# int-brain-lab/mtscomp

Hardware: AMD Instinct MI355X
Metric: compress + decompress GB/s (raw int16) (higher is better)
Workload: dtype int16

## Files before the change

mtscomp_amd/csrc/deflate.hip:

```cpp
#include <stdlib.h>

#include <mutex>

#include "deflate_dev.h"
#include "op_rank.h"

namespace mts {

#ifndef MTS_SORT_WAVES
#define MTS_SORT_WAVES 8
#endif
#ifndef MTS_SORT_KPL
#define MTS_SORT_KPL 12
#endif
constexpr int SORT_WAVES = MTS_SORT_WAVES;
constexpr int SORT_KPL = MTS_SORT_KPL;
constexpr int SORT_NT = SORT_WAVES * 64;
#ifndef MTS_SORT_B1
#define MTS_SORT_B1 7
#endif
constexpr int SORT_B1 = MTS_SORT_B1;
constexpr int SORT_B2 = 15 - SORT_B1;
#ifndef MTS_SORT_SCRAMBLE
#define MTS_SORT_SCRAMBLE 0
#endif
__device__ __forceinline__ u32 sort_hash(u32 b012)
{
    u32 h = hash_of(b012);
#if MTS_SORT_SCRAMBLE
    h ^= h >> 8;
    h = (h * 0x5bd1u) & 0x7fffu;
    h ^= h >> 7;
#endif
    return h;
}
#ifndef MTS_SORT_SWZ
#define MTS_SORT_SWZ 1
#endif
__device__ __forceinline__ u32 cslot(u32 d) { return MTS_SORT_SWZ ? d ^ (d >> 5) : d; }

template <int NB>
__device__ __forceinline__ void bin_offsets(u32 (*cnt)[256], u32 *tot)
{
    constexpr int NBIN = 1 << NB;
    const int wave = threadIdx.x >> 6, lane = threadIdx.x & 63;
    const u32 cs = cslot(threadIdx.x);
    if (threadIdx.x < NBIN) {
        u32 run = 0;
        for (int w = 0; w < SORT_WAVES; w++) { const u32 c = cnt[w][cs]; cnt[w][cs] = run; run += c; }
        tot[threadIdx.x] = run;
    }
    __syncthreads();
    if (wave == 0) {
        u32 v[4], sum = 0;
#pragma unroll
        for (int k = 0; k < 4; k++) { v[k] = (lane * 4 + k < NBIN) ? tot[lane * 4 + k] : 0; sum += v[k]; }
        u32 total;
// ... 112 lines not shown

struct OpTile;
__device__ __forceinline__ bool op_two_pass(const OpTile *ot, u32 tile);
__global__ __launch_bounds__(SORT_NT) void k_hash_sort(const u8 *__restrict__ stream, const TileDesc *__restrict__ tiles,
                                                    u32 *__restrict__ tmp, u32 *__restrict__ sorted, int lane_ordered,
                                                    const OpTile *__restrict__ only )
{
    if (only && !op_two_pass(only, blockIdx.x)) return;
    const TileDesc td = tiles[blockIdx.x];
    __shared__ u32 cnt[SORT_WAVES][256];
    __shared__ u32 cnt2[SORT_WAVES][1 << SORT_B2];
    __shared__ u32 tot[256];
    __shared__ u32 stg[SORT_WAVES * 2 * 64 * SORT_KPL];
    __shared__ u32 dlt[SORT_WAVES * 256];
    if (td.wlen == 0) return;
    const u8 *s = stream + td.stream_off + td.w;
    const u32 wlen = td.wlen;
    const int wave = threadIdx.x >> 6, lane = threadIdx.x & 63;
    const u32 per = (((wlen + SORT_WAVES - 1) / SORT_WAVES) + 63) & ~63u;
    const u32 per_magic = per > 64 ? 0xffffffffu / (per >> 6) + 1 : 0;
    for (int i = threadIdx.x; i < SORT_WAVES * 256; i += SORT_NT) (&cnt[0][0])[i] = 0;
    for (int i = threadIdx.x; i < SORT_WAVES * (1 << SORT_B2); i += SORT_NT) (&cnt2[0][0])[i] = 0;
    __syncthreads();
    {
        const u32 beg = min((u32)wave * per, wlen), end = min(beg + per, wlen);
        constexpr int CK = 8;
        if (beg < end) {
            u32 vn[CK];
#pragma unroll
            for (int k = 0; k < CK; k++) vn[k] = gld_u32_unaligned(s, min(beg + lane + 64 * k, end - 1));
            for (u32 i0 = beg + lane; i0 < end; i0 += 64 * CK) {
                u32 v[CK];
#pragma unroll
                for (int k = 0; k < CK; k++) { v[k] = vn[k]; vn[k] = gld_u32_unaligned(s, min(i0 + 64 * CK + 64 * k, end - 1)); }
#pragma unroll
                for (int k = 0; k < CK; k++) if (i0 + 64 * k < end) atomicAdd(&cnt[wave][cslot(sort_hash(v[k]) & ((1u << SORT_B1) - 1))], 1u);
            }
        }
    }
    __syncthreads();
    u32 *tmp_t = tmp + td.sorted_off, *out_t = sorted + td.sorted_off;
    auto next_counts = [&]() {
        for (int i = threadIdx.x; i < SORT_WAVES * (1 << SORT_B2); i += SORT_NT) { cnt[i >> SORT_B2][i & ((1 << SORT_B2) - 1)] = cnt2[i >> SORT_B2][i & ((1 << SORT_B2) - 1)]; cnt2[i >> SORT_B2][i & ((1 << SORT_B2) - 1)] = 0; }
        __syncthreads();
    };
    bin_offsets<SORT_B1>(cnt, tot);
    rank_pass<SORT_B1, true, 0, SORT_B2>(s, nullptr, tmp_t, wlen, per, cnt, cnt2, per_magic, lane_ordered, stg, dlt);
    next_counts();
    bin_offsets<SORT_B2>(cnt, tot);
    rank_pass<SORT_B2, false, 0, 0>(s, tmp_t, out_t, wlen, per, cnt, cnt2, per_magic, lane_ordered, stg, dlt);
}


#ifndef MTS_OP_SLICE
#define MTS_OP_SLICE 8192
#endif
constexpr int OP_SLICE = MTS_OP_SLICE;
constexpr int OP_TILE_SLICES = WIN / OP_SLICE;
#ifndef MTS_OP_WAVES
#define MTS_OP_WAVES 16
#endif
constexpr int OP_WAVES = MTS_OP_WAVES;
constexpr int OP_NT = OP_WAVES * 64;
constexpr int OP_KPL = OP_SLICE / (OP_WAVES * 64);
constexpr int OP_LMAX = 1024;
constexpr int OP_MIN_KEYS = 2 * OP_SLICE;
constexpr int OP_ROW_WORDS = 512 + 1024;
#ifndef MTS_OP_LIVE_PARTS
#define MTS_OP_LIVE_PARTS 8
#endif
constexpr int OP_LIVE_PARTS = MTS_OP_LIVE_PARTS;
struct OpTile {
    uint2 bp[1024];
    u32 live, two_pass;
    u32 pad[62];
};
__device__ __forceinline__ bool op_two_pass(const OpTile *ot, u32 tile) { return ot[tile].two_pass != 0; }
__device__ __forceinline__ u32 op_slices(u32 wlen) { return (wlen + OP_SLICE - 1) / OP_SLICE; }
__device__ __forceinline__ bool op_tile_part(int n_tiles, u32 parts, u32 &tile, u32 &part)
{
    const u32 xcd = blockIdx.x & 7, jb = blockIdx.x >> 3;
    tile = (jb / parts) * 8 + xcd; part = jb % parts;
    return tile < (u32)n_tiles;
}
static unsigned op_grid(int n_tiles, unsigned parts) { return 8u * (((unsigned)n_tiles + 7) / 8) * parts; }

typedef u32 u32x2_a4 __attribute__((ext_vector_type(2), aligned(4)));
__device__ __forceinline__ u32x2_a4 op_load8(const u8 *s, u32 p) { return *(const __attribute__((address_space(1))) u32x2_a4 *)(u64)(s + p); }
__device__ __forceinline__ u32 op_hash_at(u32x2_a4 x, int k ) { return sort_hash(k ? __builtin_amdgcn_alignbyte(x.y, x.x, (u32)k) : x.x); }

__global__ __launch_bounds__(512) void k_op_live(const u8 *__restrict__ stream, const TileDesc *__restrict__ tiles, int n_tiles, OpTile *__restrict__ ot)
{
    __shared__ u32 bm[1024];
    u32 tile, part;
    if (!op_tile_part(n_tiles, OP_LIVE_PARTS, tile, part)) return;
    const TileDesc td = tiles[tile];
    if (td.wlen < (u32)OP_MIN_KEYS) return;
    const u32 per = ((td.wlen + OP_LIVE_PARTS - 1) / OP_LIVE_PARTS + 3) & ~3u, beg = min(part * per, td.wlen), end = min(beg + per, td.wlen);
    if (beg >= end) return;
    const u8 *s = stream + td.stream_off + td.w;
    for (int i = threadIdx.x; i < 1024; i += 512) bm[i] = 0;
    __syncthreads();
    constexpr int U = 8;
    for (u32 i0 = beg + 4 * threadIdx.x; i0 < end; i0 += 4 * 512 * U) {
        u32x2_a4 v[U];
#pragma unroll
        for (int k = 0; k < U; k++) v[k] = op_load8(s, min(i0 + 4u * 512 * k, (end - 1) & ~3u));
#pragma unroll
        for (int k = 0; k < U; k++)
#pragma unroll
            for (int q = 0; q < 4; q++)
                if (i0 + 4u * 512 * k + q < end) {
                    const u32 h = op_hash_at(v[k], q), bit = 1u << (h & 31);
                    if (!(bm[h >> 5] & bit)) atomicOr(&bm[h >> 5], bit);
                }
    }
    __syncthreads();
    for (int i = threadIdx.x; i < 1024; i += 512) if (bm[i]) atomicOr(&ot[tile].bp[i].x, bm[i]);
}

__global__ __launch_bounds__(1024) void k_op_prefix(const TileDesc *__restrict__ tiles, OpTile *__restrict__ ot)
{
    __shared__ u32 wsum[16];
    const u32 tile = blockIdx.x, w = threadIdx.x;
    const u32 c = (u32)__builtin_popcount(ot[tile].bp[w].x);
    u32 tot;
    const u32 ex = wave_excl_scan_u32(c, tot);
    if ((w & 63) == 0) wsum[w >> 6] = tot;
    __syncthreads();
    u32 before = 0, all = 0;
    for (u32 q = 0; q < 16; q++) { if (q < (w >> 6)) before += wsum[q]; all += wsum[q]; }
    ot[tile].bp[w].y = before + ex;
    if (w == 0) { ot[tile].live = all; ot[tile].two_pass = (tiles[tile].wlen < (u32)OP_MIN_KEYS || all > (u32)OP_LMAX) ? 1u : 0u; }
}

__device__ __forceinline__ u32 op_bucket(const uint2 *bp, u32 h)
{
    const uint2 e = bp[h >> 5];
    return e.y + (u32)__builtin_popcount(e.x & ((1u << (h & 31)) - 1u));
}

constexpr int OP_CNT_NT = 512;
__global__ __launch_bounds__(OP_CNT_NT) void k_op_count(const u8 *__restrict__ stream, const TileDesc *__restrict__ tiles, int n_tiles,
                                                        const OpTile *__restrict__ ot, u32 *__restrict__ scratch)
{
    __shared__ uint2 bp[1024];
    __shared__ u32 cnt[OP_LMAX];
    u32 tile, slice;
    if (!op_tile_part(n_tiles, OP_TILE_SLICES, tile, slice)) return;
    if (ot[tile].two_pass) return;
    const TileDesc td = tiles[tile];
    if (slice >= op_slices(td.wlen)) return;
    const u8 *s = stream + td.stream_off + td.w;
    for (int i = threadIdx.x; i < 1024; i += OP_CNT_NT) { bp[i] = ot[tile].bp[i]; cnt[i] = 0; }
    const u32 beg = slice * OP_SLICE, end = min(beg + (u32)OP_SLICE, td.wlen);
    constexpr int U = OP_SLICE / (4 * OP_CNT_NT);
    static_assert(OP_SLICE % (4 * OP_CNT_NT) == 0, "whole loads");
    u32x2_a4 v[U];
#pragma unroll
    for (int k = 0; k < U; k++) v[k] = op_load8(s, min(beg + 4u * (OP_CNT_NT * k + threadIdx.x), (end - 1) & ~3u));
    __syncthreads();
#pragma unroll
    for (int k = 0; k < U; k++)
#pragma unroll
        for (int q = 0; q < 4; q++)
            if (beg + 4u * (OP_CNT_NT * k + threadIdx.x) + q < end) atomicAdd(&cnt[op_bucket(bp, op_hash_at(v[k], q))], 1u);
    __syncthreads();
    u16 *row = (u16 *)(scratch + td.sorted_off + (size_t)slice * OP_ROW_WORDS);
    for (int i = threadIdx.x; i < 512; i += OP_CNT_NT) ((u32 *)row)[i] = cnt[2 * i] | (cnt[2 * i + 1] << 16);
}

__global__ __launch_bounds__(1024) void k_op_scan(const TileDesc *__restrict__ tiles, const OpTile *__restrict__ ot, u32 *__restrict__ scratch)
{
    __shared__ u32 wsum[16];
    const u32 tile = blockIdx.x, b = threadIdx.x;
    if (ot[tile].two_pass) return;
    const TileDesc td = tiles[tile];
    const u32 ns = op_slices(td.wlen);
    u32 *rows = scratch + td.sorted_off;
    u32 c[OP_TILE_SLICES], total = 0;
#pragma unroll
    for (int sl = 0; sl < OP_TILE_SLICES; sl++) c[sl] = (u32)sl < ns ? ((const u16 *)(rows + (size_t)sl * OP_ROW_WORDS))[b] : 0u;
#pragma unroll
    for (int sl = 0; sl < OP_TILE_SLICES; sl++) total += c[sl];
    u32 tot;
    const u32 ex = wave_excl_scan_u32(total, tot);
    if ((b & 63) == 0) wsum[b >> 6] = tot;
    __syncthreads();
    u32 run = ex;
    for (u32 q = 0; q < (b >> 6); q++) run += wsum[q];
#pragma unroll
    for (int sl = 0; sl < OP_TILE_SLICES; sl++) {
        if ((u32)sl < ns) rows[(size_t)sl * OP_ROW_WORDS + 512 + b] = run;
        run += c[sl];
    }
}

__global__ __launch_bounds__(OP_NT) void k_op_scatter(const u8 *__restrict__ stream, const TileDesc *__restrict__ tiles, int n_tiles,
                                                    const OpTile *__restrict__ ot, const u32 *__restrict__ scratch, u32 *__restrict__ sorted)
{
    __shared__ uint2 bp[1024];
    __shared__ u32 D[OP_LMAX];
    __shared__ u32 cw[OP_WAVES][OP_LMAX / 2];
    __shared__ u32 S[OP_SLICE];
    __shared__ u32 wsum[OP_WAVES];
    static_assert(OP_LMAX <= (1 << (32 - REL_BITS)) && OP_SLICE < 65536 && OP_SLICE % (OP_WAVES * 64) == 0, "position and bucket share a word; places in a slice are 16-bit");
    u32 tile, slice;
    if (!op_tile_part(n_tiles, OP_TILE_SLICES, tile, slice)) return;
    if (ot[tile].two_pass) return;
    const TileDesc td = tiles[tile];
    if (slice >= op_slices(td.wlen)) return;
    const u8 *s = stream + td.stream_off + td.w;
    const int wave = threadIdx.x >> 6, lane = threadIdx.x & 63;
    const u32 *row = scratch + td.sorted_off + (size_t)slice * OP_ROW_WORDS;
    for (int i = threadIdx.x; i < 1024; i += OP_NT) { bp[i] = ot[tile].bp[i]; D[i] = row[512 + i]; }
    for (int i = threadIdx.x; i < OP_WAVES * (OP_LMAX / 2); i += OP_NT) (&cw[0][0])[i] = 0;
    const u32 s0 = slice * OP_SLICE, beg = s0 + (u32)wave * (OP_SLICE / OP_WAVES), end = min(s0 + (u32)OP_SLICE, td.wlen);
    u32 v[OP_KPL];
#pragma unroll
    for (int k = 0; k < OP_KPL; k++) v[k] = gld_u32_unaligned(s, min(beg + 64u * k + lane, td.wlen - 1));
    __syncthreads();
    static_assert(OP_LMAX <= (1 << OP_ID_BITS) && OP_KPL * 64 <= (1 << (32 - OP_ID_BITS)), "bucket and rank share a word");
    u32 idr[OP_KPL];
#pragma unroll
    for (int k = 0; k < OP_KPL; k++) {
        const u32 id = op_bucket(bp, sort_hash(v[k]));
        idr[k] = id;
        if (beg + 64u * k + lane < end) idr[k] = op_pack_rank(id, atomicAdd(&cw[wave][op_cw_word(id)], op_cw_one(id)));
    }
    __syncthreads();
    {
        const int j = threadIdx.x & (OP_LMAX / 2 - 1);
        const bool mine = threadIdx.x < OP_LMAX / 2;
        u32 c[OP_WAVES], tot = 0;
#pragma unroll
        for (int w = 0; w < OP_WAVES; w++) { c[w] = mine ? cw[w][j] : 0u; tot += c[w]; }
        const u32 c0 = tot & 0xffffu, c1 = tot >> 16;
        u32 wtot;
        const u32 ex = wave_excl_scan_u32(c0 + c1, wtot);
        if (lane == 0) wsum[wave] = wtot;
        __syncthreads();
        u32 st0 = ex;
        for (int w = 0; w < wave; w++) st0 += wsum[w];
        const u32 st1 = st0 + c0;
        u32 run = st0 | (st1 << 16);
        if (mine) {
#pragma unroll
// ... 12 lines not shown
        }
    }
    __syncthreads();
    u32 *out = sorted + td.sorted_off;
    const u32 nk = end - s0;
#pragma unroll
    for (int k = 0; k < OP_KPL; k++) {
        const u32 j = threadIdx.x + (u32)OP_NT * k;
        if (j < nk) { const u32 e = S[j]; out[D[e >> REL_BITS] + j] = e; }
    }
}

static int lds_lane_ordered()
{
    static std::mutex mu;
    static int cached[64];
    static bool init = false;
    std::lock_guard<std::mutex> lk(mu);
    if (!init) { for (int i = 0; i < 64; i++) cached[i] = -1; init = true; }
    int dev = 0;
    if (hipGetDevice(&dev) != hipSuccess || dev < 0 || dev >= 64) return 0;
    if (cached[dev] >= 0) return cached[dev];
    u32 *d_bad = nullptr, h_bad = 1;
    if (hipMalloc(&d_bad, 4) != hipSuccess) return 0;
    if (hipMemset(d_bad, 0, 4) == hipSuccess) {
        hipLaunchKernelGGL(k_probe_lds_order, dim3(64), dim3(1024), 0, 0, d_bad, 512);
        if (hipMemcpy(&h_bad, d_bad, 4, hipMemcpyDeviceToHost) != hipSuccess) h_bad = 1;
    }
    (void)hipFree(d_bad);
    cached[dev] = h_bad == 0 ? 1 : 0;
    return cached[dev];
}

__global__ void k_inject_disorder(const u8 *__restrict__ stream, const TileDesc *__restrict__ tiles, u32 *__restrict__ sorted)
{
    const TileDesc td = tiles[0];
    const u8 *s = stream + td.stream_off + td.w;
    u32 *sk = sorted + td.sorted_off;
    for (u32 i = 0; i + 1 < td.wlen; i++) {
        const u32 a = sk[i], b = sk[i + 1];
        if (hash_of(gld_u32_unaligned(s, a & REL_MASK)) == hash_of(gld_u32_unaligned(s, b & REL_MASK)) && (b & REL_MASK) >= td.a - td.w) { sk[i] = b; sk[i + 1] = a; return; }
    }
}

size_t hash_sort_ws_bytes(int n_tiles) { return (size_t)(n_tiles + 1) * sizeof(OpTile); }

int launch_hash_sort(hipStream_t st, const u8 *d_stream, const TileDesc *d_tiles, int n_tiles, u32 *d_tmp, u32 *d_sorted, int force_ballot, void *d_ws)
{
    if (n_tiles == 0) return MTS_OK;
    const int ordered = (force_ballot == 1 || getenv("MTS_SORT_BALLOT")) ? 0 : lds_lane_ordered();
    static const bool two_pass_only = getenv("MTS_SORT_TWO_PASS") != nullptr;
    if (ordered && d_ws && !two_pass_only) {
        OpTile *ot = (OpTile *)d_ws;
        MTS_HIP(hipMemsetAsync(ot, 0, sizeof(OpTile) * (size_t)n_tiles, st));
        hipLaunchKernelGGL(k_op_live, dim3(op_grid(n_tiles, OP_LIVE_PARTS)), dim3(512), 0, st, d_stream, d_tiles, n_tiles, ot);
        hipLaunchKernelGGL(k_op_prefix, dim3(n_tiles), dim3(1024), 0, st, d_tiles, ot);
        hipLaunchKernelGGL(k_hash_sort, dim3(n_tiles), dim3(SORT_NT), 0, st, d_stream, d_tiles, d_tmp, d_sorted, ordered, (const OpTile *)ot);
        hipLaunchKernelGGL(k_op_count, dim3(op_grid(n_tiles, OP_TILE_SLICES)), dim3(OP_CNT_NT), 0, st, d_stream, d_tiles, n_tiles, (const OpTile *)ot, d_tmp);
        hipLaunchKernelGGL(k_op_scan, dim3(n_tiles), dim3(1024), 0, st, d_tiles, (const OpTile *)ot, d_tmp);
        hipLaunchKernelGGL(k_op_scatter, dim3(op_grid(n_tiles, OP_TILE_SLICES)), dim3(OP_NT), 0, st, d_stream, d_tiles, n_tiles, (const OpTile *)ot, (const u32 *)d_tmp, d_sorted);
    } else
        hipLaunchKernelGGL(k_hash_sort, dim3(n_tiles), dim3(SORT_NT), 0, st, d_stream, d_tiles, d_tmp, d_sorted, ordered, (const OpTile *)nullptr);
    if (force_ballot == 2) hipLaunchKernelGGL(k_inject_disorder, dim3(1), dim3(1), 0, st, d_stream, d_tiles, d_sorted);
    MTS_HIP(hipGetLastError());
    return MTS_OK;
}


typedef u32 u32x4_v __attribute__((ext_vector_type(4)));
typedef u32 u32x4_a4 __attribute__((ext_vector_type(4), aligned(4)));
typedef const __attribute__((address_space(1))) u32 *gptr_u32c;
typedef const __attribute__((address_space(1))) u32x4_v *gptr_uint4;
typedef const __attribute__((address_space(1))) u32x4_a4 *gptr_uint4_a4;
template <bool AHEAD, class RDU, class RD, class RDQ>
__device__ __forceinline__ u32 lazy_step(RDU &&rdu , RD &&rd, RDQ &&rdq, u32 p0, u32 n, const LevelCfg &cfg, u32 &mpos, u32 &mlen, u32 &mdist,
                                         u32 &mside )
{
    u32 p = p0;
    mside = 0;
    const u32 e0 = rdu(p);
    u32 e1 = 0, e2 = 0, e3 = 0;
    if (AHEAD) { e1 = rdu(p + 1); e2 = rdu(p + 2); e3 = rdu(p + 3); }
    u32 len = te_len(e0), dist = te_dist(e0);
    if (len == MIN_MATCH && dist > (u32)TOO_FAR) len = 0;
    if (len < MIN_MATCH) { mpos = p0; mlen = 0; mdist = 0; return p0 + 1; }
    for (;;) {
        const u32 q = p + 1;
        if (q < n && len < (u32)cfg.lazy) {
            u32 d;
            if (AHEAD) { d = q == p0 + 1 ? e1 : q == p0 + 2 ? e2 : e3; if (q > p0 + 3) d = rd(q); }
            else d = rd(q);
            u32 side = 0;
            if (len >= (u32)cfg.good) {
                if (d & TE_QNONE) d = 0;
                else if (d & TE_QSIDE) { d = rdq(q); side = 1; }
            }
            const u32 dl = te_len(d);
            if (dl > len) { p = q; len = dl; dist = te_dist(d); mside = side; continue; }
        }
        break;
    }
    mpos = p; mlen = len; mdist = dist;
    return p + len;
}
#define MTS_PARSE_GLOBAL_READERS(T, TQ)                                 \
    auto rd = [&](u32 q) -> u32 { return (T)[q]; };                     \
    auto rdq = [&](u32 q) -> u32 { return (TQ)[q]; };

constexpr int PARSE_WIN = 32;
constexpr int PARSE_AHEAD = 4;
constexpr int PARSE_ROW = PARSE_WIN + PARSE_AHEAD;
constexpr int PARSE_WIN_PITCH = PARSE_ROW + 1;
// ... 1636 lines not shown
```

mtscomp_amd/csrc/transform.hip:

```cpp
#include <stdlib.h>

#include "common.h"

namespace mts {


__device__ __forceinline__ u64 wave_sum_u64(u64 v)
{
#pragma unroll
    for (int off = 32; off > 0; off >>= 1) {
        u32 lo = __shfl_down((u32)v, off, 64), hi = __shfl_down((u32)(v >> 32), off, 64);
        v += ((u64)hi << 32) | lo;
    }
    return v;
}

__device__ __forceinline__ void block_sum2(u64 &a, u64 &b, u64 *sh )
{
    a = wave_sum_u64(a);
    b = wave_sum_u64(b);
    const int wave = threadIdx.x >> 6, lane = threadIdx.x & 63, nw = blockDim.x >> 6;
    if (lane == 0) { sh[wave] = a; sh[4 + wave] = b; }
    __syncthreads();
    if (threadIdx.x == 0) {
// ... 647 lines not shown
                const u32 v = (tt < tt_rows && t0 + tt < nt) ? (u32)d[(u64)c * nt + t0 + tt] : 0u;
                const u32 x = wave_incl_scan_dpp32(v) + run;
                if (tt < tt_rows) tile[tt * pitch + c] = (T)x;
                run = (u32)__builtin_amdgcn_readlane((int)x, 63);
            }
        }
    }
    __syncthreads();
    const int nrow = (int)min((long)tt_rows, nt - t0);
    T *out = (T *)(outb + out_off[chunk]) + t0 * nc;
    const long e_n = (long)nrow * nc;
    if ((((u64)out) & 15) == 0 && sizeof(T) <= 4) {
        constexpr int VW = 16 / (int)sizeof(T);
        const long n_full = e_n / VW;
        uint4 *oq = (uint4 *)out;
        for (long i = threadIdx.x; i < n_full; i += 256) {
            u32 r = __umulhi((u32)i * VW, nc_magic), c = (u32)i * VW - r * nc;
            u32 w[4] = {0, 0, 0, 0};
#pragma unroll
            for (int j = 0; j < VW; j++) {
                w[j / EPD] |= (u32)tile[r * pitch + c] << (8 * sizeof(T) * (j % EPD));
                if (++c == (u32)nc) { c = 0; r++; }
            }
            oq[i] = make_uint4(w[0], w[1], w[2], w[3]);
        }
        for (long e = n_full * VW + threadIdx.x; e < e_n; e += 256) {
            const u32 r = __umulhi((u32)e, nc_magic), c = (u32)e - r * nc;
            out[e] = tile[r * pitch + c];
        }
    } else if ((((u64)out) & 3) == 0) {
        u32 *od = (u32 *)out;
        for (long i = threadIdx.x; i * EPD < e_n; i += 256) {
            u32 v = 0;
            bool full = true;
#pragma unroll
            for (int j = 0; j < EPD; j++) {
                const u32 e = (u32)i * EPD + j;
                if (e < e_n) {
                    const u32 r = __umulhi(e, nc_magic), c = e - r * nc;
                    v |= (u32)tile[r * pitch + c] << (8 * sizeof(T) * j);
                } else full = false;
            }
            if (full) od[i] = v;
            else for (int j = 0; j < EPD; j++) if ((long)i * EPD + j < e_n) out[i * EPD + j] = (T)(v >> (8 * sizeof(T) * j));
        }
    } else {
        for (long i = threadIdx.x; i < e_n; i += 256) {
            const u32 r = __umulhi((u32)i, nc_magic), c = (u32)i - r * nc;
            out[i] = tile[r * pitch + c];
        }
    }
}

template <typename T>
static int run_cumsum_rows(hipStream_t st, const u8 *stream, u8 *out, const u64 *d_stream_off, const u64 *d_out_off,
                            const u32 *d_rows, const int *d_status, int n_chunks, u32 max_rows, int nc, u32 *sums)
{
    const int tt = rows_tile(nc, (int)sizeof(T)), pitch = rows_pitch(nc, (int)sizeof(T));
    const size_t lds = (size_t)tt * pitch * sizeof(T);
    const int rc = ensure_dynamic_lds((const void *)k_cumsum_rows<T>, ROWS_LDS_LIMIT);
    if (rc) return rc;
    const int ntile = (max_rows + tt - 1) / tt;
    dim3 grid(xcd_row_grid(ntile, n_chunks));
    hipLaunchKernelGGL(k_rows_sums<T>, grid, dim3(256), 0, st, stream, d_stream_off, d_rows, d_status, nc, tt, ntile, sums);
    hipLaunchKernelGGL(k_rows_scan, dim3((nc + 63) / 64, n_chunks), dim3(64 * ROWS_SCAN_PARTS), 0, st, d_rows, d_status, nc, tt, ntile, sums);
    hipLaunchKernelGGL(k_cumsum_rows<T>, grid, dim3(256), lds, st, stream, out, d_stream_off, d_out_off, d_rows, d_status, nc, tt, pitch,
                       0xffffffffu / (u32)nc + 1, ntile, sums);
    return MTS_OK;
}

static int segr_for(int itemsize) { return itemsize <= 2 ? 256 : itemsize == 4 ? 128 : 64; }

size_t cumsum_scratch_bytes(int n_chunks, u32 max_rows, int n_channels)
{
    const size_t seg = (size_t)n_chunks * ((max_rows + 63) / 64 + 1) * n_channels * sizeof(u64);
    const size_t til = (size_t)n_chunks * ((max_rows + 15) / 16 + 1) * n_channels * sizeof(u32);
    return (seg > til ? seg : til) + 256;
}

int launch_cumsum_transpose(hipStream_t st, const void *d_stream, void *d_out, const u64 *d_stream_off,
                            const u64 *d_out_off, const u32 *d_rows, const int *d_status, int n_chunks,
                            u32 max_rows, int n_channels, int itemsize, int flags, void *d_segsums)
{
    if (n_chunks == 0 || max_rows == 0) return MTS_OK;
    const u8 *s = (const u8 *)d_stream;
    u8 *o = (u8 *)d_out;
    u64 *ss = (u64 *)d_segsums;
    (void)segr_for;
    if (flags & MTS_FLAG_FLOAT) {
        if (itemsize == 4) return run_cumsum_float<float>(st, s, o, d_stream_off, d_out_off, d_rows, d_status, n_chunks, max_rows, n_channels, flags);
        if (itemsize == 8) return run_cumsum_float<double>(st, s, o, d_stream_off, d_out_off, d_rows, d_status, n_chunks, max_rows, n_channels, flags);
        return MTS_E_ARG;
    }
    if (flags == (MTS_FLAG_TIME_DIFF | MTS_FLAG_ORDER_F) && itemsize <= 4 && n_channels >= 2 && rows_tile(n_channels, itemsize) && !getenv("MTS_K12_GENERIC")) {
        int rc;
        switch (itemsize) {
        case 1: rc = run_cumsum_rows<u8>(st, s, o, d_stream_off, d_out_off, d_rows, d_status, n_chunks, max_rows, n_channels, (u32 *)ss); break;
        case 2: rc = run_cumsum_rows<u16>(st, s, o, d_stream_off, d_out_off, d_rows, d_status, n_chunks, max_rows, n_channels, (u32 *)ss); break;
        default: rc = run_cumsum_rows<u32>(st, s, o, d_stream_off, d_out_off, d_rows, d_status, n_chunks, max_rows, n_channels, (u32 *)ss); break;
        }
        if (rc) return rc;
        MTS_HIP(hipGetLastError());
        return MTS_OK;
    }
    switch (itemsize) {
    case 1: return run_cumsum<u8, 256>(st, s, o, d_stream_off, d_out_off, d_rows, d_status, n_chunks, max_rows, n_channels, flags, ss);
    case 2: return run_cumsum<u16, 256>(st, s, o, d_stream_off, d_out_off, d_rows, d_status, n_chunks, max_rows, n_channels, flags, ss);
    case 4: return run_cumsum<u32, 128>(st, s, o, d_stream_off, d_out_off, d_rows, d_status, n_chunks, max_rows, n_channels, flags, ss);
    case 8: return run_cumsum<u64, 64>(st, s, o, d_stream_off, d_out_off, d_rows, d_status, n_chunks, max_rows, n_channels, flags, ss);
    default: return MTS_E_ARG;
// ... 92 lines not shown
```

Before: 36.11.

## Fuse live-bitmap, prefix, count and scan into one per-tile planner kernel

Replaces four kernels plus a memset (k_op_live, k_op_prefix, k_op_count, k_op_scan) with a single k_op_plan that builds the live-hash bitmap, prefixes it, counts per-slice bucket occupancy in LDS with 16-bit packed counters, and writes the slice offsets for the scatter. It also computes hash word/bit directly from the key without the full sort_hash when scrambling is off, and software-pipelines the loads. This removes launch overhead and global round-trips for bitmap and count rows. In exchange each tile is handled by only one 1024-thread block, so there is less parallelism than the old slice-parallel count, and a large dynamic LDS footprint limits occupancy.

```diff
diff --git a/mtscomp_amd/csrc/deflate.hip b/mtscomp_amd/csrc/deflate.hip
--- a/mtscomp_amd/csrc/deflate.hip
+++ b/mtscomp_amd/csrc/deflate.hip
@@ -3,6 +3,7 @@
 #include <mutex>
 
 #include "deflate_dev.h"
+#include "op_plan.h"
 #include "op_rank.h"
 
 namespace mts {
@@ -221,31 +222,19 @@
 }
 
 
-#ifndef MTS_OP_SLICE
-#define MTS_OP_SLICE 8192
-#endif
-constexpr int OP_SLICE = MTS_OP_SLICE;
-constexpr int OP_TILE_SLICES = WIN / OP_SLICE;
 #ifndef MTS_OP_WAVES
 #define MTS_OP_WAVES 16
 #endif
 constexpr int OP_WAVES = MTS_OP_WAVES;
 constexpr int OP_NT = OP_WAVES * 64;
 constexpr int OP_KPL = OP_SLICE / (OP_WAVES * 64);
-constexpr int OP_LMAX = 1024;
 constexpr int OP_MIN_KEYS = 2 * OP_SLICE;
-constexpr int OP_ROW_WORDS = 512 + 1024;
-#ifndef MTS_OP_LIVE_PARTS
-#define MTS_OP_LIVE_PARTS 8
-#endif
-constexpr int OP_LIVE_PARTS = MTS_OP_LIVE_PARTS;
 struct OpTile {
     uint2 bp[1024];
     u32 live, two_pass;
     u32 pad[62];
 };
 __device__ __forceinline__ bool op_two_pass(const OpTile *ot, u32 tile) { return ot[tile].two_pass != 0; }
-__device__ __forceinline__ u32 op_slices(u32 wlen) { return (wlen + OP_SLICE - 1) / OP_SLICE; }
 __device__ __forceinline__ bool op_tile_part(int n_tiles, u32 parts, u32 &tile, u32 &part)
 {
     const u32 xcd = blockIdx.x & 7, jb = blockIdx.x >> 3;
@@ -258,110 +247,154 @@
 __device__ __forceinline__ u32x2_a4 op_load8(const u8 *s, u32 p) { return *(const __attribute__((address_space(1))) u32x2_a4 *)(u64)(s + p); }
 __device__ __forceinline__ u32 op_hash_at(u32x2_a4 x, int k ) { return sort_hash(k ? __builtin_amdgcn_alignbyte(x.y, x.x, (u32)k) : x.x); }
 
-__global__ __launch_bounds__(512) void k_op_live(const u8 *__restrict__ stream, const TileDesc *__restrict__ tiles, int n_tiles, OpTile *__restrict__ ot)
-{
-    __shared__ u32 bm[1024];
-    u32 tile, part;
-    if (!op_tile_part(n_tiles, OP_LIVE_PARTS, tile, part)) return;
-    const TileDesc td = tiles[tile];
-    if (td.wlen < (u32)OP_MIN_KEYS) return;
-    const u32 per = ((td.wlen + OP_LIVE_PARTS - 1) / OP_LIVE_PARTS + 3) & ~3u, beg = min(part * per, td.wlen), end = min(beg + per, td.wlen);
-    if (beg >= end) return;
-    const u8 *s = stream + td.stream_off + td.w;
-    for (int i = threadIdx.x; i < 1024; i += 512) bm[i] = 0;
-    __syncthreads();
-    constexpr int U = 8;
-    for (u32 i0 = beg + 4 * threadIdx.x; i0 < end; i0 += 4 * 512 * U) {
-        u32x2_a4 v[U];
-#pragma unroll
-        for (int k = 0; k < U; k++) v[k] = op_load8(s, min(i0 + 4u * 512 * k, (end - 1) & ~3u));
-#pragma unroll
-        for (int k = 0; k < U; k++)
-#pragma unroll
-            for (int q = 0; q < 4; q++)
-                if (i0 + 4u * 512 * k + q < end) {
-                    const u32 h = op_hash_at(v[k], q), bit = 1u << (h & 31);
-                    if (!(bm[h >> 5] & bit)) atomicOr(&bm[h >> 5], bit);
-                }
-    }
-    __syncthreads();
-    for (int i = threadIdx.x; i < 1024; i += 512) if (bm[i]) atomicOr(&ot[tile].bp[i].x, bm[i]);
-}
-
-__global__ __launch_bounds__(1024) void k_op_prefix(const TileDesc *__restrict__ tiles, OpTile *__restrict__ ot)
-{
-    __shared__ u32 wsum[16];
-    const u32 tile = blockIdx.x, w = threadIdx.x;
-    const u32 c = (u32)__builtin_popcount(ot[tile].bp[w].x);
-    u32 tot;
-    const u32 ex = wave_excl_scan_u32(c, tot);
-    if ((w & 63) == 0) wsum[w >> 6] = tot;
-    __syncthreads();
-    u32 before = 0, all = 0;
-    for (u32 q = 0; q < 16; q++) { if (q < (w >> 6)) before += wsum[q]; all += wsum[q]; }
-    ot[tile].bp[w].y = before + ex;
-    if (w == 0) { ot[tile].live = all; ot[tile].two_pass = (tiles[tile].wlen < (u32)OP_MIN_KEYS || all > (u32)OP_LMAX) ? 1u : 0u; }
-}
-
 __device__ __forceinline__ u32 op_bucket(const uint2 *bp, u32 h)
 {
     const uint2 e = bp[h >> 5];
     return e.y + (u32)__builtin_popcount(e.x & ((1u << (h & 31)) - 1u));
 }
 
-constexpr int OP_CNT_NT = 512;
-__global__ __launch_bounds__(OP_CNT_NT) void k_op_count(const u8 *__restrict__ stream, const TileDesc *__restrict__ tiles, int n_tiles,
-                                                        const OpTile *__restrict__ ot, u32 *__restrict__ scratch)
-{
-    __shared__ uint2 bp[1024];
-    __shared__ u32 cnt[OP_LMAX];
-    u32 tile, slice;
-    if (!op_tile_part(n_tiles, OP_TILE_SLICES, tile, slice)) return;
-    if (ot[tile].two_pass) return;
+template <int SH>
+__device__ __forceinline__ u32 op_hash_word_off(u32 y)
+{
+#if MTS_SORT_SCRAMBLE
+    return (sort_hash(y) >> 5) << SH;
+#else
+    static_assert(SH <= 5, "c2's upper three bits are shifted down");
+    return ((y << (5 + SH)) ^ (((y >> 8) & 0xffu) << SH) ^ (((y >> 16) & 0xffu) >> (5 - SH))) & (0x3ffu << SH);
+#endif
+}
+__device__ __forceinline__ u32 op_hash_bit(u32 y) { return MTS_SORT_SCRAMBLE ? sort_hash(y) & 31u : (y >> 16) & 31u; }
+__device__ __forceinline__ u32 op_key_at(u32x2_a4 x, int k ) { return k ? __builtin_amdgcn_alignbyte(x.y, x.x, (u32)k) : x.x; }
+
+constexpr int OP_PLAN_U = 4;
+template <bool FULL>
+__device__ __forceinline__ void op_plan_mark_step(u32 *bm, const u32x2_a4 (&v)[OP_PLAN_U], u32 p0, u32 stride, u32 wlen)
+{
+#pragma unroll
+    for (int k = 0; k < OP_PLAN_U; k++) {
+        u32 *at[4], bit[4], w[4];
+#pragma unroll
+        for (int q = 0; q < 4; q++) {
+            const u32 y = op_key_at(v[k], q);
+            at[q] = (u32 *)((u8 *)bm + op_hash_word_off<2>(y)); bit[q] = 1u << op_hash_bit(y); w[q] = *at[q];
+        }
+#pragma unroll
+        for (int q = 0; q < 4; q++)
+            if ((FULL || p0 + stride * k + q < wlen) && !(w[q] & bit[q])) atomicOr(at[q], bit[q]);
+    }
+}
+template <bool FULL>
+__device__ __forceinline__ void op_plan_count_step(u32 *cnt_row , u32 one , const uint2 *bp, const u32x2_a4 (&v)[OP_PLAN_U], u32 p0, u32 wlen)
+{
+#pragma unroll
+    for (int k = 0; k < OP_PLAN_U; k++) {
+        u32 id[4];
+#pragma unroll
+        for (int q = 0; q < 4; q++) {
+            const u32 y = op_key_at(v[k], q);
+            const uint2 e = *(const uint2 *)((const u8 *)bp + op_hash_word_off<3>(y));
+            id[q] = e.y + (u32)__builtin_popcount(e.x & ((1u << op_hash_bit(y)) - 1u));
+        }
+#pragma unroll
+        for (int q = 0; q < 4; q++)
+            if (FULL || p0 + 256u * k + q < wlen) atomicAdd(&cnt_row[id[q]], one);
+    }
+}
+
+constexpr int OP_PLAN_NT = OP_PLAN_WAVES * 64;
+constexpr int OP_PLAN_CNT_WORDS = OP_PLAN_ROWS * OP_LMAX;
+constexpr int OP_PLAN_DYN_LDS = OP_PLAN_CNT_WORDS * 4;
+constexpr int OP_PLAN_LDS = OP_PLAN_DYN_LDS + 1024 * 4 + 1024 * 8 + OP_PLAN_WAVES * 4;
+static_assert(OP_PLAN_NT == 1024 && OP_LMAX == OP_PLAN_NT && (OP_SLICE / 256) % OP_PLAN_U == 0, "a thread per word of the bitmap, and a thread per bucket");
+static_assert(OP_PLAN_LDS <= (REL_BITS == 18 ? 80 : 160) * 1024, "two planners share a CU's 160 KB (one, with the 2^19 window)");
+
+__global__ __launch_bounds__(OP_PLAN_NT, 8) void k_op_plan(const u8 *__restrict__ stream, const TileDesc *__restrict__ tiles, int n_tiles,
+                                                           OpTile *__restrict__ ot, u32 *__restrict__ scratch)
+{
+    struct {
+        u32 *bm;
+        uint2 *bp;
+        u32 *wsum, *cnt;
+    } L;
+    __shared__ u32 s_bm[1024];
+    __shared__ uint2 s_bp[1024];
+    __shared__ u32 s_wsum[OP_PLAN_WAVES];
+    extern __shared__ __attribute__((aligned(16))) u8 smem[];
+    L.bm = s_bm; L.bp = s_bp; L.wsum = s_wsum; L.cnt = (u32 *)smem;
+    u32 tile, part;
+    if (!op_tile_part(n_tiles, 1, tile, part)) return;
     const TileDesc td = tiles[tile];
-    if (slice >= op_slices(td.wlen)) return;
+    const u32 wlen = td.wlen, t = threadIdx.x, wave = (u32)__builtin_amdgcn_readfirstlane((int)(t >> 6)), lane = t & 63;
+    if (wlen < (u32)OP_MIN_KEYS) {
+        if (t == 0) { ot[tile].live = 0; ot[tile].two_pass = 1u; }
+        return;
+    }
     const u8 *s = stream + td.stream_off + td.w;
-    for (int i = threadIdx.x; i < 1024; i += OP_CNT_NT) { bp[i] = ot[tile].bp[i]; cnt[i] = 0; }
-    const u32 beg = slice * OP_SLICE, end = min(beg + (u32)OP_SLICE, td.wlen);
-    constexpr int U = OP_SLICE / (4 * OP_CNT_NT);
-    static_assert(OP_SLICE % (4 * OP_CNT_NT) == 0, "whole loads");
-    u32x2_a4 v[U];
-#pragma unroll
-    for (int k = 0; k < U; k++) v[k] = op_load8(s, min(beg + 4u * (OP_CNT_NT * k + threadIdx.x), (end - 1) & ~3u));
-    __syncthreads();
-#pragma unroll
-    for (int k = 0; k < U; k++)
-#pragma unroll
-        for (int q = 0; q < 4; q++)
-            if (beg + 4u * (OP_CNT_NT * k + threadIdx.x) + q < end) atomicAdd(&cnt[op_bucket(bp, op_hash_at(v[k], q))], 1u);
-    __syncthreads();
-    u16 *row = (u16 *)(scratch + td.sorted_off + (size_t)slice * OP_ROW_WORDS);
-    for (int i = threadIdx.x; i < 512; i += OP_CNT_NT) ((u32 *)row)[i] = cnt[2 * i] | (cnt[2 * i + 1] << 16);
-}
-
-__global__ __launch_bounds__(1024) void k_op_scan(const TileDesc *__restrict__ tiles, const OpTile *__restrict__ ot, u32 *__restrict__ scratch)
-{
-    __shared__ u32 wsum[16];
-    const u32 tile = blockIdx.x, b = threadIdx.x;
-    if (ot[tile].two_pass) return;
-    const TileDesc td = tiles[tile];
-    const u32 ns = op_slices(td.wlen);
-    u32 *rows = scratch + td.sorted_off;
-    u32 c[OP_TILE_SLICES], total = 0;
-#pragma unroll
-    for (int sl = 0; sl < OP_TILE_SLICES; sl++) c[sl] = (u32)sl < ns ? ((const u16 *)(rows + (size_t)sl * OP_ROW_WORDS))[b] : 0u;
-#pragma unroll
-    for (int sl = 0; sl < OP_TILE_SLICES; sl++) total += c[sl];
-    u32 tot;
-    const u32 ex = wave_excl_scan_u32(total, tot);
-    if ((b & 63) == 0) wsum[b >> 6] = tot;
-    __syncthreads();
-    u32 run = ex;
-    for (u32 q = 0; q < (b >> 6); q++) run += wsum[q];
-#pragma unroll
-    for (int sl = 0; sl < OP_TILE_SLICES; sl++) {
-        if ((u32)sl < ns) rows[(size_t)sl * OP_ROW_WORDS + 512 + b] = run;
-        run += c[sl];
+    constexpr int U = OP_PLAN_U;
+    L.bm[t] = 0;
+    for (int i = t; i < OP_PLAN_CNT_WORDS; i += OP_PLAN_NT) L.cnt[i] = 0;
+    __syncthreads();
+    {
+        constexpr u32 STRIDE = 4u * OP_PLAN_NT, STEP = STRIDE * U;
+        const u32 nst = (wlen + STEP - 1) / STEP;
+        u32x2_a4 vn[U];
+#pragma unroll
+        for (int k = 0; k < U; k++) vn[k] = op_load8(s, op_plan_load_at(4 * t + STRIDE * k, wlen));
+        for (u32 st = 0; st < nst; st++) {
+            const u32 p0 = STEP * st + 4 * t;
+            u32x2_a4 v[U];
+#pragma unroll
+            for (int k = 0; k < U; k++) { v[k] = vn[k]; vn[k] = op_load8(s, op_plan_load_at(p0 + STEP + STRIDE * k, wlen)); }
+            if (STEP * (st + 1) <= wlen) op_plan_mark_step<true>(L.bm, v, p0, STRIDE, wlen);
+            else op_plan_mark_step<false>(L.bm, v, p0, STRIDE, wlen);
+        }
+    }
+    __syncthreads();
+    {
+        const u32 m = L.bm[t];
+        u32 tot;
+        const u32 ex = wave_excl_scan_u32((u32)__builtin_popcount(m), tot);
+        if (lane == 0) L.wsum[wave] = tot;
+        __syncthreads();
+        u32 before = 0, all = 0;
+        for (u32 q = 0; q < (u32)OP_PLAN_WAVES; q++) { if (q < wave) before += L.wsum[q]; all += L.wsum[q]; }
+        const uint2 e = make_uint2(m, before + ex);
+        L.bp[t] = e;
+        ot[tile].bp[t] = e;
+        const bool two_pass = all > (u32)OP_LMAX;
+        if (t == 0) { ot[tile].live = all; ot[tile].two_pass = two_pass ? 1u : 0u; }
+        if (t < 62) ot[tile].pad[t] = 0;
+        if (two_pass) return;
+        __syncthreads();
+    }
+    const u32 ns = op_slices(wlen);
+    {
+        constexpr u32 SPS = (u32)OP_SLICE / 256 / U;
+        u32 nj = 0;
+        while (op_plan_wave_slice(wave, nj) < ns) nj++;
+        const u32 nst = nj * SPS;
+        auto pos = [&](u32 st, int k) { return op_plan_pos(op_plan_wave_slice(wave, st / SPS), (st % SPS) * U + k, lane); };
+        u32x2_a4 vn[U];
+#pragma unroll
+        for (int k = 0; k < U; k++) vn[k] = op_load8(s, op_plan_load_at(pos(0, k), wlen));
+        for (u32 st = 0; st < nst; st++) {
+            u32x2_a4 v[U];
+#pragma unroll
+            for (int k = 0; k < U; k++) { v[k] = vn[k]; vn[k] = op_load8(s, op_plan_load_at(pos(st + 1, k), wlen)); }
+            const u32 sl = op_plan_wave_slice(wave, st / SPS), first = op_plan_pos(sl, (st % SPS) * U, 0);
+            if (first + 256u * U <= wlen) op_plan_count_step<true>(L.cnt + op_plan_word(sl, 0), op_plan_one(sl), L.bp, v, first + 4 * lane, wlen);
+            else if (first < wlen) op_plan_count_step<false>(L.cnt + op_plan_word(sl, 0), op_plan_one(sl), L.bp, v, first + 4 * lane, wlen);
+        }
+    }
+    __syncthreads();
+    {
+        u32 tot;
+        const u32 ex = wave_excl_scan_u32(op_plan_total(L.cnt, ns, t), tot);
+        if (lane == 0) L.wsum[wave] = tot;
+        __syncthreads();
+        u32 start = ex;
+        for (u32 q = 0; q < wave; q++) start += L.wsum[q];
+        op_plan_offsets(L.cnt, ns, t, start, scratch + td.sorted_off);
     }
 }
 
@@ -480,12 +513,9 @@
     static const bool two_pass_only = getenv("MTS_SORT_TWO_PASS") != nullptr;
     if (ordered && d_ws && !two_pass_only) {
         OpTile *ot = (OpTile *)d_ws;
-        MTS_HIP(hipMemsetAsync(ot, 0, sizeof(OpTile) * (size_t)n_tiles, st));
-        hipLaunchKernelGGL(k_op_live, dim3(op_grid(n_tiles, OP_LIVE_PARTS)), dim3(512), 0, st, d_stream, d_tiles, n_tiles, ot);
-        hipLaunchKernelGGL(k_op_prefix, dim3(n_tiles), dim3(1024), 0, st, d_tiles, ot);
+        MTS_LDS_ATTR(k_op_plan, OP_PLAN_LDS);
+        hipLaunchKernelGGL(k_op_plan, dim3(op_grid(n_tiles, 1)), dim3(OP_PLAN_NT), OP_PLAN_DYN_LDS, st, d_stream, d_tiles, n_tiles, ot, d_tmp);
         hipLaunchKernelGGL(k_hash_sort, dim3(n_tiles), dim3(SORT_NT), 0, st, d_stream, d_tiles, d_tmp, d_sorted, ordered, (const OpTile *)ot);
-        hipLaunchKernelGGL(k_op_count, dim3(op_grid(n_tiles, OP_TILE_SLICES)), dim3(OP_CNT_NT), 0, st, d_stream, d_tiles, n_tiles, (const OpTile *)ot, d_tmp);
-        hipLaunchKernelGGL(k_op_scan, dim3(n_tiles), dim3(1024), 0, st, d_tiles, (const OpTile *)ot, d_tmp);
         hipLaunchKernelGGL(k_op_scatter, dim3(op_grid(n_tiles, OP_TILE_SLICES)), dim3(OP_NT), 0, st, d_stream, d_tiles, n_tiles, (const OpTile *)ot, (const u32 *)d_tmp, d_sorted);
     } else
         hipLaunchKernelGGL(k_hash_sort, dim3(n_tiles), dim3(SORT_NT), 0, st, d_stream, d_tiles, d_tmp, d_sorted, ordered, (const OpTile *)nullptr);
diff --git a/mtscomp_amd/csrc/op_plan.h b/mtscomp_amd/csrc/op_plan.h
--- /dev/null
+++ b/mtscomp_amd/csrc/op_plan.h
@@ -0,0 +1,48 @@
+#pragma once
+#include <stddef.h>
+#include <stdint.h>
+
+#include "codec_plan.h"
+#include "op_rank.h"
+
+#ifndef MTS_OP_SLICE
+#define MTS_OP_SLICE 8192
+#endif
+
+namespace mts {
+
+constexpr int OP_SLICE = MTS_OP_SLICE;
+constexpr int OP_LMAX = 1024;
+constexpr int OP_ROW_WORDS = 512 + 1024;
+constexpr int OP_PLAN_WAVES = 16;
+constexpr int OP_TILE_SLICES = WIN / OP_SLICE;
+constexpr int OP_PLAN_ROWS = OP_TILE_SLICES / 2;
+static_assert(OP_SLICE < 65536, "a 16-bit half holds a slice's keys of one bucket, all of them at the most: it never carries into its neighbour");
+static_assert(OP_SLICE % 256 == 0, "a wave's 8-byte loads (four positions a lane) cover a slice in whole instructions");
+static_assert(OP_TILE_SLICES % 2 == 0 && OP_PLAN_ROWS % OP_PLAN_WAVES == 0, "wave w counts the slices w, w + 16, ..: with those the rows w, w + 16, .. and no others");
+
+OP_RANK_FN uint32_t op_slices(uint32_t wlen) { return (wlen + OP_SLICE - 1) / OP_SLICE; }
+OP_RANK_FN uint32_t op_slice_of(uint32_t pos) { return pos / OP_SLICE; }
+OP_RANK_FN uint32_t op_plan_wave_slice(uint32_t wave, uint32_t j) { return wave + (uint32_t)OP_PLAN_WAVES * j; }
+OP_RANK_FN uint32_t op_plan_pos(uint32_t slice, uint32_t k, uint32_t lane) { return slice * (uint32_t)OP_SLICE + 4u * (64u * k + lane); }
+OP_RANK_FN uint32_t op_plan_load_at(uint32_t pos, uint32_t wlen) { const uint32_t last = (wlen - 1u) & ~3u; return pos < last ? pos : last; }
+OP_RANK_FN uint32_t op_plan_shift(uint32_t slice) { return 16u * (slice / (uint32_t)OP_PLAN_ROWS); }
+OP_RANK_FN uint32_t op_plan_one(uint32_t slice) { return 1u << op_plan_shift(slice); }
+OP_RANK_FN uint32_t op_plan_word(uint32_t slice, uint32_t id) { return (slice % (uint32_t)OP_PLAN_ROWS) * (uint32_t)OP_LMAX + id; }
+OP_RANK_FN uint32_t op_plan_count(const uint32_t *cnt, uint32_t slice, uint32_t id) { return (cnt[op_plan_word(slice, id)] >> op_plan_shift(slice)) & 0xffffu; }
+OP_RANK_FN uint32_t op_plan_total(const uint32_t *cnt, uint32_t n_slices, uint32_t id)
+{
+    uint32_t t = 0;
+    for (uint32_t sl = 0; sl < n_slices; sl++) t += op_plan_count(cnt, sl, id);
+    return t;
+}
+OP_RANK_FN void op_plan_offsets(const uint32_t *cnt, uint32_t n_slices, uint32_t id, uint32_t start, uint32_t *rows)
+{
+    uint32_t run = start;
+    for (uint32_t sl = 0; sl < n_slices; sl++) {
+        rows[(size_t)sl * OP_ROW_WORDS + 512 + id] = run;
+        run += op_plan_count(cnt, sl, id);
+    }
+}
+
+}
```

Result: no change. 36.35 (median of 6 runs) (+0.7%).

## Add single-pass column-strip cumsum kernel replacing three-launch row-tile scan

Applied to the files above, without the earlier changes.

Adds a k_cumsum_strips kernel in which each block owns a strip of channels for one chunk. It walks time tiles sequentially, carrying running sums in registers, prefetches D tiles ahead, scans within the wave using DPP, and transposes through double-buffered LDS before writing with buffer stores. This replaces the three-kernel sums/scan/apply pipeline with one pass over the data, dropping the extra read of the input. Strips are picked automatically when there are enough chunk×strip blocks per CU. The cost is serial dependence along time inside each block and more complex edge handling.

```diff
diff --git a/mtscomp_amd/csrc/transform.hip b/mtscomp_amd/csrc/transform.hip
--- a/mtscomp_amd/csrc/transform.hip
+++ b/mtscomp_amd/csrc/transform.hip
@@ -723,10 +723,229 @@
     }
 }
 
+#ifndef MTS_K2_STRIPS_D
+#define MTS_K2_STRIPS_D 3
+#endif
+#ifndef MTS_K2_STRIPS_THREADS
+#define MTS_K2_STRIPS_THREADS 512
+#endif
+constexpr int STRIP_TT = 64;
+constexpr int STRIP_THREADS = MTS_K2_STRIPS_THREADS;
+constexpr int STRIP_MAX_SLOTS = 8;
+__host__ __device__ constexpr int strip_cps(int itemsize) { return STRIP_THREADS / (STRIP_TT / (8 / itemsize)); }
+__host__ __device__ inline int strip_pitch(int w, int itemsize)
+{
+    const int ipl = 8 / itemsize, u = (w + 2 * ipl - 2) / ipl;
+    return (u | 1) * ipl;
+}
+static int strip_width(int nc, int itemsize)
+{
+    const int w0 = 4 * strip_cps(itemsize) - (8 / itemsize - 1), nstrip = (nc + w0 - 1) / w0;
+    return (nc + nstrip - 1) / nstrip;
+}
+#ifndef MTS_K2_STRIPS_MIN_PER_CU_X4
+#define MTS_K2_STRIPS_MIN_PER_CU_X4 3
+#endif
+static int strips_for_batch(int n_chunks, int nc, int itemsize, int n_cu)
+{
+    const int w = strip_width(nc, itemsize), nstrip = (nc + w - 1) / w;
+    return 4L * n_chunks * nstrip >= (long)MTS_K2_STRIPS_MIN_PER_CU_X4 * n_cu ? w : 0;
+}
+__device__ __forceinline__ bool xcd_chunk_strip(int nstrip, int n_chunks, int &chunk, int &strip)
+{
+    const u32 xcd = blockIdx.x & 7, j = blockIdx.x >> 3;
+    chunk = (int)(j / (u32)nstrip * 8 + xcd);
+    strip = (int)(j % (u32)nstrip);
+    return chunk < n_chunks;
+}
+static unsigned xcd_strip_grid(int nstrip, int n_chunks) { return 8u * (((unsigned)n_chunks + 7) / 8) * (unsigned)nstrip; }
+
+typedef u32 strip_v2 __attribute__((ext_vector_type(2)));
+__device__ __forceinline__ void strip_store_item(u8 v, __amdgpu_buffer_rsrc_t rs, int off) { __builtin_amdgcn_raw_buffer_store_b8(v, rs, off, 0, 0); }
+__device__ __forceinline__ void strip_store_item(u16 v, __amdgpu_buffer_rsrc_t rs, int off) { __builtin_amdgcn_raw_buffer_store_b16(v, rs, off, 0, 0); }
+__device__ __forceinline__ void strip_store_item(u32 v, __amdgpu_buffer_rsrc_t rs, int off) { __builtin_amdgcn_raw_buffer_store_b32(v, rs, off, 0, 0); }
+
+template <typename T, int NS, bool FAST>
+__device__ __forceinline__ void strips_walk(const T *__restrict__ d, T *__restrict__ out, T *lds, long nt, int nc, int c0, int wn, int pitch)
+{
+    constexpr int TT = STRIP_TT, D = MTS_K2_STRIPS_D;
+    constexpr int SZ = (int)sizeof(T), EPD = 4 / SZ, IPL = 8 / SZ, LPC = TT / IPL, CPS = strip_cps(SZ);
+    constexpr int LPR = NS * CPS / IPL, RPI = STRIP_THREADS / LPR;
+    constexpr int KI = (TT * 2 * (IPL - 1) + STRIP_THREADS - 1) / STRIP_THREADS;
+    const int tid = threadIdx.x, lane = tid & 63, q = tid % LPC, cs = tid / LPC;
+    const int ntile = (int)((nt + TT - 1) / TT);
+    const u32 pb = (u32)((u64)out / SZ) + (u32)c0;
+    auto load = [&](int k, uint2 (&w)[NS]) {
+        const long t = (long)k * TT + q * IPL;
+#pragma unroll
+        for (int s = 0; s < NS; s++) {
+            const int cl = s * CPS + cs;
+            if (FAST) w[s] = *(const uint2 *)(d + (u64)(c0 + min(cl, wn - 1)) * (u64)nt + min(t, nt - IPL));
+            else {
+                u32 ww[2] = {0u, 0u};
+                if (cl < wn) {
+                    const T *p = d + (u64)(c0 + cl) * (u64)nt + t;
+#pragma unroll
+                    for (int j = 0; j < IPL; j++) if (t + j < nt) ww[j / EPD] |= (u32)p[j] << (8 * SZ * (j % EPD));
+                }
+                w[s] = make_uint2(ww[0], ww[1]);
+            }
+        }
+    };
+    uint2 wq[D][NS], wn_q[D][NS];
+    u32 carry[NS];
+#pragma unroll
+    for (int s = 0; s < NS; s++) carry[s] = 0u;
+#pragma unroll
+    for (int dd = 0; dd < D; dd++) load(dd, wq[dd]);
+#pragma unroll
+    for (int dd = 0; dd < D; dd++)
+#pragma unroll
+        for (int s = 0; s < NS; s++) asm volatile("" : "+v"(wq[dd][s].x), "+v"(wq[dd][s].y));
+    constexpr int NOWHERE = 0x7ffffff0;
+    const u32 mis = (u32)((u64)out & 7);
+    int wofs[IPL];
+#pragma unroll
+    for (int j = 0; j < IPL; j++) wofs[j] = (q * IPL + j) * pitch + cs + (int)((pb + (u32)(q * IPL + j) * (u32)nc) & (IPL - 1));
+    int rd8[TT / RPI], st8[TT / RPI], rdi[KI], sti[KI];
+    {
+        const int l = tid % LPR, r0 = tid / LPR;
+#pragma unroll
+        for (int i = 0; i < TT / RPI; i++) {
+            const int r = i * RPI + r0;
+            const u32 b0 = mis + (u32)(r * nc + c0) * SZ;
+            const int lo = l * IPL - (int)(b0 & 7) / SZ;
+            rd8[i] = r * pitch + min(l, pitch / IPL - 1) * IPL;
+            st8[i] = lo >= 0 && lo + IPL <= wn ? (int)((b0 & ~7u) + 8u * l) : NOWHERE;
+        }
+#pragma unroll
+        for (int m = 0; m < KI; m++) {
+            const int idx = tid + STRIP_THREADS * m, r = idx / (2 * (IPL - 1)), pos = idx - r * (2 * (IPL - 1));
+            const bool tail = pos >= IPL - 1;
+            const int e = tail ? pos - (IPL - 1) : pos;
+            const u32 b0 = mis + (u32)(r * nc + c0) * SZ;
+            const int ph = (int)(b0 & 7) / SZ;
+            const int hn = min(wn, (IPL - ph) % IPL), tn = min((ph + wn) % IPL, wn - hn);
+            const bool ok = r < TT && (tail ? e < tn : e < hn);
+            const int it = ok ? (tail ? wn - tn + e : e) : 0;
+            rdi[m] = min(r, TT - 1) * pitch + ph + it;
+            sti[m] = ok ? (int)(b0 + (u32)it * SZ) : NOWHERE;
+        }
+    }
+    for (int k0 = 0; k0 < ntile; k0 += D) {
+#pragma unroll
+        for (int dd = 0; dd < D; dd++) load(k0 + D + dd, wn_q[dd]);
+#pragma unroll
+        for (int dd = 0; dd < D; dd++) {
+            const int k = k0 + dd;
+            uint2 cur[NS];
+#pragma unroll
+            for (int s = 0; s < NS; s++) cur[s] = wq[dd][s];
+            T *tile = lds + (size_t)(k & 1) * TT * pitch;
+            const long t0 = (long)k * TT;
+#pragma unroll
+            for (int s = 0; s < NS; s++) {
+                const u32 ww[2] = {cur[s].x, cur[s].y};
+                u32 x[IPL], tot = 0, add;
+#pragma unroll
+                for (int j = 0; j < IPL; j++) { tot += (u32)(T)(ww[j / EPD] >> (8 * SZ * (j % EPD))); x[j] = tot; }
+                if constexpr (LPC == 16) {
+                    u32 sc = tot, rt = tot;
+                    sc += (u32)__builtin_amdgcn_update_dpp(0, (int)sc, 0x111, 0xf, 0xf, false);
+                    sc += (u32)__builtin_amdgcn_update_dpp(0, (int)sc, 0x112, 0xf, 0xf, false);
+                    sc += (u32)__builtin_amdgcn_update_dpp(0, (int)sc, 0x114, 0xf, 0xf, false);
+                    sc += (u32)__builtin_amdgcn_update_dpp(0, (int)sc, 0x118, 0xf, 0xf, false);
+                    rt += (u32)__builtin_amdgcn_update_dpp(0, (int)rt, 0x128, 0xf, 0xf, false);
+                    rt += (u32)__builtin_amdgcn_update_dpp(0, (int)rt, 0x124, 0xf, 0xf, false);
+                    rt += (u32)__builtin_amdgcn_update_dpp(0, (int)rt, 0x122, 0xf, 0xf, false);
+                    rt += (u32)__builtin_amdgcn_update_dpp(0, (int)rt, 0x121, 0xf, 0xf, false);
+                    add = carry[s] + sc - tot;
+                    carry[s] += rt;
+                } else {
+                    const u32 v = wave_incl_scan_dpp32(tot);
+                    const u32 prev = (u32)__shfl((int)v, (lane - q - 1) & 63, 64);
+                    const u32 last = (u32)__shfl((int)v, lane - q + LPC - 1, 64);
+                    const u32 before = (lane - q) ? prev : 0u;
+                    add = carry[s] + v - tot - before;
+                    carry[s] += last - before;
+                }
+                if (s * CPS + cs < wn) {
+#pragma unroll
+                    for (int j = 0; j < IPL; j++) tile[wofs[j] + s * CPS] = (T)(x[j] + add);
+                }
+            }
+            __syncthreads();
+            const int nrow = (int)max(0L, min((long)TT, nt - t0));
+            const __amdgpu_buffer_rsrc_t rs = __builtin_amdgcn_make_buffer_rsrc((u8 *)(out + (u64)t0 * (u64)nc) - mis, 0, (int)(mis + (u32)nrow * (u32)nc * SZ), 0x00020000);
+            uint2 v[TT / RPI];
+            T vi[KI];
+#pragma unroll
+            for (int i = 0; i < TT / RPI; i++) v[i] = *(const uint2 *)(tile + rd8[i]);
+#pragma unroll
+            for (int m = 0; m < KI; m++) vi[m] = tile[rdi[m]];
+#pragma unroll
+            for (int i = 0; i < TT / RPI; i++) __builtin_amdgcn_raw_buffer_store_b64(strip_v2{v[i].x, v[i].y}, rs, st8[i], 0, 0);
+#pragma unroll
+            for (int m = 0; m < KI; m++) strip_store_item(vi[m], rs, sti[m]);
+        }
+#pragma unroll
+        for (int dd = 0; dd < D; dd++)
+#pragma unroll
+            for (int s = 0; s < NS; s++) wq[dd][s] = wn_q[dd][s];
+    }
+}
+
+template <typename T, int NS>
+__global__ __launch_bounds__(STRIP_THREADS) void k_cumsum_strips(const u8 *__restrict__ stream, u8 *__restrict__ outb,
+                                                       const u64 *__restrict__ stream_off, const u64 *__restrict__ out_off,
+                                                       const u32 *__restrict__ rows, const int *__restrict__ status,
+                                                       int nc, int n_chunks, int w, int nstrip, int pitch)
+{
+    extern __shared__ __attribute__((aligned(16))) u8 smem_rows[];
+    int chunk, strip;
+    if (!xcd_chunk_strip(nstrip, n_chunks, chunk, strip)) return;
+    if (status && status[chunk] != 0) return;
+    const long nt = rows[chunk];
+    if (nt == 0) return;
+    const int c0 = strip * w, wn = min(w, nc - c0);
+    const T *d = (const T *)(stream + stream_off[chunk]);
+    T *out = (T *)(outb + out_off[chunk]);
+    if (((u64)nt * sizeof(T)) % 8 == 0 && (((u64)d) & 7) == 0) strips_walk<T, NS, true>(d, out, (T *)smem_rows, nt, nc, c0, wn, pitch);
+    else strips_walk<T, NS, false>(d, out, (T *)smem_rows, nt, nc, c0, wn, pitch);
+}
+
+template <typename T>
+static int run_cumsum_strips(hipStream_t st, const u8 *stream, u8 *out, const u64 *d_stream_off, const u64 *d_out_off,
+                             const u32 *d_rows, const int *d_status, int n_chunks, int nc, int w)
+{
+    constexpr int CPS = strip_cps((int)sizeof(T));
+    w = w < nc ? w : nc;
+    constexpr int IPL = 8 / (int)sizeof(T);
+    if (w > STRIP_MAX_SLOTS * CPS - (IPL - 1)) w = STRIP_MAX_SLOTS * CPS - (IPL - 1);
+    if (w > 46 * IPL + 1) w = 46 * IPL + 1;
+    const int nstrip = (nc + w - 1) / w, slots = (w + IPL - 1 + CPS - 1) / CPS, pitch = strip_pitch(w, (int)sizeof(T));
+    const size_t lds = (size_t)2 * STRIP_TT * pitch * sizeof(T);
+    const dim3 grid(xcd_strip_grid(nstrip, n_chunks));
+    if (slots <= 2) hipLaunchKernelGGL((k_cumsum_strips<T, 2>), grid, dim3(STRIP_THREADS), lds, st, stream, out, d_stream_off, d_out_off, d_rows, d_status, nc, n_chunks, w, nstrip, pitch);
+    else if (slots <= 4) hipLaunchKernelGGL((k_cumsum_strips<T, 4>), grid, dim3(STRIP_THREADS), lds, st, stream, out, d_stream_off, d_out_off, d_rows, d_status, nc, n_chunks, w, nstrip, pitch);
+    else hipLaunchKernelGGL((k_cumsum_strips<T, STRIP_MAX_SLOTS>), grid, dim3(STRIP_THREADS), lds, st, stream, out, d_stream_off, d_out_off, d_rows, d_status, nc, n_chunks, w, nstrip, pitch);
+    return MTS_OK;
+}
+
+static int strips_choice(int n_chunks, int nc, int itemsize)
+{
+    if (const char *e = getenv("MTS_K2_STRIPS")) { const int n = atoi(e); return n > 0 ? n : 0; }
+    int dev = 0, n_cu = 0;
+    if (hipGetDevice(&dev) != hipSuccess || hipDeviceGetAttribute(&n_cu, hipDeviceAttributeMultiprocessorCount, dev) != hipSuccess || n_cu <= 0) return 0;
+    return strips_for_batch(n_chunks, nc, itemsize, n_cu);
+}
+
 template <typename T>
 static int run_cumsum_rows(hipStream_t st, const u8 *stream, u8 *out, const u64 *d_stream_off, const u64 *d_out_off,
                             const u32 *d_rows, const int *d_status, int n_chunks, u32 max_rows, int nc, u32 *sums)
 {
+    if (const int w = strips_choice(n_chunks, nc, (int)sizeof(T)))
+        return run_cumsum_strips<T>(st, stream, out, d_stream_off, d_out_off, d_rows, d_status, n_chunks, nc, w);
     const int tt = rows_tile(nc, (int)sizeof(T)), pitch = rows_pitch(nc, (int)sizeof(T));
     const size_t lds = (size_t)tt * pitch * sizeof(T);
     const int rc = ensure_dynamic_lds((const void *)k_cumsum_rows<T>, ROWS_LDS_LIMIT);
```

Measured after the change: 36.37 before, 36.60 after, median of 6. About the same (+0.6%).
